# nanoporetech/medaka

Measured on NVIDIA H100. Metric: pileup positions/sec (consensus inference), higher is better.
Workload: dtype f32

## Files before the change

### medaka_b200/csrc/gru_wg.cu

```cuda
#include "common.cuh"
#include "ptx.cuh"
#include "rec_common.cuh"

namespace mdk {

constexpr int RW_THREADS = 256;
constexpr int RW_ABLK = (H / 8) * 64 * 16;
constexpr int RW_XBLK = 2 * 64 * 16;

template <int NT, bool FUSE_X, int OUT>
struct RwCfg {
    static constexpr int N = NT * RT_N;
    static constexpr bool HL = NT == 1;
    static constexpr int ROWS = HL ? 2 * N : N;
    static constexpr int PLANES = HL ? 1 : 2;
    static constexpr int KG = ROWS * 16 + 16;
    static constexpr int HPLANE = (H / 8) * KG;
    static constexpr int XPLANE = 2 * KG;
    static constexpr int HLO = HL ? N * 16 : HPLANE;
    static constexpr int XLO = HL ? N * 16 : XPLANE;
    static constexpr int RED = (RW_THREADS / 32) * NCLS * N;
    static constexpr int wlo_off = 0;
    static constexpr int wxlo_off = wlo_off + 6 * RW_ABLK;
    static constexpr int h_off = wxlo_off + (FUSE_X ? 6 * RW_XBLK : 0);
    static constexpr int x_off = h_off + 2 * PLANES * HPLANE;
    static constexpr int red_off = x_off + (FUSE_X ? 2 * PLANES * XPLANE : 0);
    static constexpr int total = red_off + (OUT == OUT_LOGITS ? 2 * RED * 4 : 0);
    static_assert(total <= 227 * 1024, "smem budget");
};

__device__ __forceinline__ uint32_t ld_u32(const __half *p) { return *reinterpret_cast<const uint32_t *>(p); }

template <int NT, bool FUSE_X, int OUT>
__global__ void __launch_bounds__(RW_THREADS, 1)
rec_tc_kernel(const float *__restrict__ gi, RecX xin, const __half *__restrict__ w_hh, const float *__restrict__ b_hn,
              void *__restrict__ h_out, int64_t B, int64_t T, const float *__restrict__ lin_w,
              float *__restrict__ plog) {
    using L = RwCfg<NT, FUSE_X, OUT>;
    constexpr int N = L::N, NA = N / 2;
    constexpr int NACC = L::ROWS / 2;
    constexpr int NX = FUSE_X ? NACC : NA;
    using MMA = Wgmma<N>;
    using MMA_H = Wgmma<L::ROWS>;
    constexpr bool LOGITS = OUT == OUT_LOGITS;
    extern __shared__ __align__(128) uint8_t smem[];
    const int tid = threadIdx.x, wg = tid >> 7, warp = (tid >> 5) & 3, lane = tid & 31;
    const int gq = lane >> 2, cq = lane & 3;
    const int dir = blockIdx.y;
    const int64_t ntiles = (B + RT_N - 1) / RT_N;
    const int64_t wtile0 = (int64_t)blockIdx.x * NT;
    const int j0 = wg * 64 + warp * 16 + gq;
    const uint32_t sbase = smem_u32(smem);

    for (int i = tid; i < (L::total - L::h_off) / 16; i += RW_THREADS)
        reinterpret_cast<int4 *>(smem + L::h_off)[i] = make_int4(0, 0, 0, 0);
    for (int i = tid; i < 3 * H * (H / 8); i += RW_THREADS) {
        const int kg = i & 15, r = (i >> 4) & (H - 1), gate = i >> 11;
        const uint4 v = *reinterpret_cast<const uint4 *>(w_hh + ((((size_t)dir * 2 + 1) * 3 + gate) * H + r) * H + kg * 8);
        *reinterpret_cast<uint4 *>(smem + L::wlo_off + (gate * 2 + (r >> 6)) * RW_ABLK + kg * 1024 + (r & 63) * 16) = v;
    }
    if (FUSE_X) {
        for (int i = tid; i < 3 * H * 2; i += RW_THREADS) {
            const int kg = i & 1, r = (i >> 1) & (H - 1), gate = i >> 8;
            const uint4 v = *reinterpret_cast<const uint4 *>(xin.w_x + ((((size_t)dir * 2 + 1) * 3 + gate) * H + r) * 16 + kg * 8);
            *reinterpret_cast<uint4 *>(smem + L::wxlo_off + (gate * 2 + (r >> 6)) * RW_XBLK + kg * 1024 + (r & 63) * 16) = v;
        }
    }
    float wlin[2][NCLS];
    if (LOGITS) {
#pragma unroll
        for (int hb = 0; hb < 2; ++hb)
#pragma unroll
            for (int c = 0; c < NCLS; ++c) wlin[hb][c] = lin_w[c * H2 + dir * H + j0 + 8 * hb];
    }
    uint32_t whi[3][H / 16][4];
#pragma unroll
    for (int gate = 0; gate < 3; ++gate)
#pragma unroll
        for (int ks = 0; ks < H / 16; ++ks) {
            const __half *w = w_hh + ((((size_t)dir * 2) * 3 + gate) * H + j0) * H + ks * 16 + 2 * cq;
            whi[gate][ks][0] = ld_u32(w);
            whi[gate][ks][1] = ld_u32(w + 8 * H);
            whi[gate][ks][2] = ld_u32(w + 8);
            whi[gate][ks][3] = ld_u32(w + 8 * H + 8);
        }
    uint32_t wxhi[3][4];
    float bx[3][2] = {};
    if (FUSE_X) {
#pragma unroll
        for (int gate = 0; gate < 3; ++gate) {
            const __half *w = xin.w_x + ((((size_t)dir * 2) * 3 + gate) * H + j0) * 16 + 2 * cq;
            wxhi[gate][0] = ld_u32(w);
            wxhi[gate][1] = ld_u32(w + 8 * 16);
            wxhi[gate][2] = ld_u32(w + 8);
            wxhi[gate][3] = ld_u32(w + 8 * 16 + 8);
            bx[gate][0] = xin.bias[dir * G3 + gate * H + j0];
            bx[gate][1] = xin.bias[dir * G3 + gate * H + j0 + 8];
        }
    }
    const float bhn[2] = {b_hn[dir * H + j0], b_hn[dir * H + j0 + 8]};

    float ar[NACC], az[NACC], an[NACC], axn[NX], hp[NA];
#pragma unroll
    for (int k = 0; k < NA; ++k) hp[k] = 0.f;
    auto load_pre = [&](int64_t t) {
#pragma unroll
        for (int i = 0; i < N / 8; ++i)
#pragma unroll
            for (int hb = 0; hb < 2; ++hb) {
                float2 v[3] = {make_float2(0.f, 0.f), make_float2(0.f, 0.f), make_float2(0.f, 0.f)};
                if (FUSE_X) {
#pragma unroll
                    for (int gate = 0; gate < 3; ++gate) v[gate] = make_float2(bx[gate][hb], bx[gate][hb]);
                } else if (wtile0 + (i >> 1) < ntiles) {
                    const float *p = gi + ((wtile0 + (i >> 1)) * T + t) * GI_TS_FLOATS +
                                     (((dir * 3) * 4 + 2 * (i & 1) + (cq >> 1)) * H + j0 + 8 * hb) * 4 + 2 * (cq & 1);
#pragma unroll
                    for (int gate = 0; gate < 3; ++gate) v[gate] = __ldcs(reinterpret_cast<const float2 *>(p + gate * 16 * H));
                }
                const int k = 4 * i + 2 * hb;
                ar[k] = v[0].x; ar[k + 1] = v[0].y;
                az[k] = v[1].x; az[k + 1] = v[1].y;
                axn[k] = v[2].x; axn[k + 1] = v[2].y;
                an[k] = bhn[hb]; an[k + 1] = bhn[hb];
            }
        if constexpr (L::HL) {
#pragma unroll
            for (int k = NA; k < NACC; ++k) {
                ar[k] = 0.f; az[k] = 0.f; an[k] = 0.f;
                if constexpr (FUSE_X) axn[k] = 0.f;
            }
        }
    };
    const int xF = FUSE_X ? xin.F : 1;
    const float *xsrc[NT];
    int xoff[NT];
    float xreg[NT];
#pragma unroll
    for (int m = 0; m < NT; ++m) {
        const int q = tid + RW_THREADS * m, xn = q / xF, xf = q - xn * xF;
        const bool own = FUSE_X && q < N * xF;
        xoff[m] = own ? (xf >> 3) * L::KG + xn * 16 + (xf & 7) * 2 : -1;
        xsrc[m] = (own && wtile0 * RT_N + xn < B) ? xin.feats + ((wtile0 * RT_N + xn) * T) * xF + xf : nullptr;
        xreg[m] = 0.f;
    }
    auto stage_x = [&](int buf, int m, float v) {
        __half hi, lo;
        split_f16(v, hi, lo);
        *reinterpret_cast<__half *>(smem + L::x_off + buf * L::PLANES * L::XPLANE + xoff[m]) = hi;
        *reinterpret_cast<__half *>(smem + L::x_off + buf * L::PLANES * L::XPLANE + L::XLO + xoff[m]) = lo;
    };
    const int64_t t_first = dir ? T - 1 : 0;
    if (FUSE_X) {
#pragma unroll
        for (int m = 0; m < NT; ++m) {
            if (xoff[m] < 0) continue;
            stage_x(0, m, xsrc[m] ? xsrc[m][t_first * xF] : 0.f);
            if (xsrc[m] && T > 1) xreg[m] = xsrc[m][(dir ? T - 2 : 1) * xF];
        }
    }
    load_pre(t_first);
    fence_proxy_async_smem();
    __syncthreads();

    constexpr int NW = N / 4;
    auto head_partials = [&](int rb) {
        float v[NW][NCLS];
#pragma unroll
        for (int wl = 0; wl < NW; ++wl) {
            const int k = 4 * (wl >> 1) + (wl & 1);
#pragma unroll
            for (int c = 0; c < NCLS; ++c) v[wl][c] = fmaf(wlin[1][c], hp[k + 2], wlin[0][c] * hp[k]);
        }
        int wbase = 0;
#pragma unroll
        for (int lvl = 0; lvl < 3; ++lvl) {
            const int mask = 16 >> lvl;
            const int half = (NW >> lvl) / 2;
            if (half > 0) {
                const bool up = lane & mask;
#pragma unroll
                for (int w = 0; w < NW / 2; ++w) {
                    if (w >= half) continue;
#pragma unroll
                    for (int c = 0; c < NCLS; ++c) {
                        const float send = up ? v[w][c] : v[w + half][c];
                        const float keep = up ? v[w + half][c] : v[w][c];
                        v[w][c] = keep + __shfl_xor_sync(0xffffffffu, send, mask);
                    }
                }
                if (up) wbase += half;
            } else {
#pragma unroll
                for (int c = 0; c < NCLS; ++c) v[0][c] += __shfl_xor_sync(0xffffffffu, v[0][c], mask);
            }
        }
        if (NW >= 8 || !(lane & 4)) {
            float *red = reinterpret_cast<float *>(smem + L::red_off) + rb * L::RED + (tid >> 5) * NCLS * N;
            const int n = 8 * (wbase >> 1) + 2 * cq + (wbase & 1);
#pragma unroll
            for (int c = 0; c < NCLS; ++c) red[c * N + n] = v[0][c];
        }
    };
    auto head_store = [&](int rb, int64_t t) {
        if (tid >= NCLS * N) return;
        const int c = tid / N, n = tid % N;
        const float *red = reinterpret_cast<const float *>(smem + L::red_off) + rb * L::RED + c * N + n;
        float s = red[0];
#pragma unroll
        for (int w = 1; w < RW_THREADS / 32; ++w) s += red[w * NCLS * N];
        const int64_t wt = wtile0 + n / RT_N;
        if (wt < ntiles) plog[((dir * ntiles + wt) * T + t) * PLOG_TS_FLOATS + c * RT_N + (n & 15)] = s;
    };

#pragma unroll 1
    for (int64_t step = 0; step < T; ++step) {
        const int64_t t = dir ? T - 1 - step : step;
        const int buf = (int)(step & 1);
        const uint32_t hb_addr = sbase + L::h_off + buf * L::PLANES * L::HPLANE;
        wg_fence();
        if constexpr (L::HL) {
#pragma unroll
            for (int ks = 0; ks < H / 16; ++ks) {
                const uint64_t bh = make_smem_desc(hb_addr + ks * 2 * L::KG, L::KG, 128);
#pragma unroll
                for (int gate = 0; gate < 3; ++gate) MMA_H::rs(gate == 0 ? ar : (gate == 1 ? az : an), whi[gate][ks], bh, 1u);
#pragma unroll
                for (int gate = 0; gate < 3; ++gate)
                    MMA::ss(gate == 0 ? ar : (gate == 1 ? az : an),
                            make_smem_desc(sbase + L::wlo_off + (gate * 2 + wg) * RW_ABLK + ks * 2 * 1024, 1024, 128), bh, 1u);
            }
        } else {
#pragma unroll
            for (int gate = 0; gate < 3; ++gate) {
                float(&acc)[NACC] = gate == 0 ? ar : (gate == 1 ? az : an);
#pragma unroll
                for (int ks = 0; ks < H / 16; ++ks) {
                    const uint64_t bh = make_smem_desc(hb_addr + ks * 2 * L::KG, L::KG, 128);
                    MMA::rs(acc, whi[gate][ks], bh, 1u);
                    MMA::rs(acc, whi[gate][ks], make_smem_desc(hb_addr + L::HPLANE + ks * 2 * L::KG, L::KG, 128), 1u);
                    MMA::ss(acc, make_smem_desc(sbase + L::wlo_off + (gate * 2 + wg) * RW_ABLK + ks * 2 * 1024, 1024, 128), bh, 1u);
                }
            }
        }
        if constexpr (FUSE_X) {
            const uint32_t xa = sbase + L::x_off + buf * L::PLANES * L::XPLANE;
            const uint64_t bh = make_smem_desc(xa, L::KG, 128);
            if constexpr (L::HL) {
#pragma unroll
                for (int gate = 0; gate < 3; ++gate) MMA_H::rs(gate == 0 ? ar : (gate == 1 ? az : axn), wxhi[gate], bh, 1u);
#pragma unroll
                for (int gate = 0; gate < 3; ++gate)
                    MMA::ss(gate == 0 ? ar : (gate == 1 ? az : axn),
                            make_smem_desc(sbase + L::wxlo_off + (gate * 2 + wg) * RW_XBLK, 1024, 128), bh, 1u);
            } else {
                const uint64_t bl = make_smem_desc(xa + L::XPLANE, L::KG, 128);
#pragma unroll
                for (int gate = 0; gate < 3; ++gate) {
                    float(&acc)[NACC] = gate == 0 ? ar : (gate == 1 ? az : axn);
                    MMA::rs(acc, wxhi[gate], bh, 1u);
                    MMA::rs(acc, wxhi[gate], bl, 1u);
                    MMA::ss(acc, make_smem_desc(sbase + L::wxlo_off + (gate * 2 + wg) * RW_XBLK, 1024, 128), bh, 1u);
                }
            }
        }
        wg_commit();
        if (!FUSE_X && tid == 0 && step + GI_PREFETCH_STEPS < T) {
            const int64_t tp = dir ? t - GI_PREFETCH_STEPS : t + GI_PREFETCH_STEPS;
#pragma unroll
            for (int m = 0; m < NT; ++m) {
                if (wtile0 + m >= ntiles) break;
                const float *blk = gi + ((wtile0 + m) * T + tp) * GI_TS_FLOATS + (int64_t)dir * (GI_TS_FLOATS / 2);
#pragma unroll
                for (int i = 0; i < 12; ++i) bulk_prefetch_l2(blk + i * 512, 2048);
            }
        }
        if (LOGITS && step > 0) {
            if (step > 1) head_store((int)((step - 1) & 1), dir ? t + 2 : t - 2);
            head_partials((int)(step & 1));
        }
        wg_wait_all();
        wg_hold(ar); wg_hold(az); wg_hold(an); wg_hold(axn);

        uint8_t *hw = smem + L::h_off + (buf ^ 1) * L::PLANES * L::HPLANE;
#pragma unroll
        for (int k = 0; k < NA; ++k) {
            float pr = ar[k], pz = az[k], pn = an[k], px = axn[k], r, z;
            if constexpr (L::HL) {
                pr += ar[k + NA]; pz += az[k + NA]; pn += an[k + NA];
                if constexpr (FUSE_X) px += axn[k + NA];
                const float a = 1.f + ex2_approx(fminf(pr, EXP_CLAMP)), b = 1.f + ex2_approx(fminf(pz, EXP_CLAMP));
                const float q = rcp_approx(a * b);
                r = b * q;
                z = a * q;
            } else {
                r = rcp_approx(1.f + ex2_approx(fminf(pr, EXP_CLAMP)));
                z = rcp_approx(1.f + ex2_approx(fminf(pz, EXP_CLAMP)));
            }
            const float en = ex2_approx(fminf(fmaf(r, pn, px), EXP_CLAMP));
            const float n = (en - 1.f) * rcp_approx(en + 1.f);
            hp[k] = fmaf(z, hp[k] - n, n);
            const int j = j0 + 8 * ((k >> 1) & 1), col = 8 * (k >> 2) + 2 * cq + (k & 1);
            __half hi, lo;
            split_f16(hp[k], hi, lo);
            *reinterpret_cast<__half *>(hw + (j >> 3) * L::KG + col * 16 + (j & 7) * 2) = hi;
            *reinterpret_cast<__half *>(hw + L::HLO + (j >> 3) * L::KG + col * 16 + (j & 7) * 2) = lo;
        }
        if (FUSE_X && step + 1 < T) {
#pragma unroll
            for (int m = 0; m < NT; ++m) {
                if (xoff[m] < 0) continue;
                stage_x(buf ^ 1, m, xreg[m]);
                if (xsrc[m] && step + 2 < T) xreg[m] = xsrc[m][(dir ? t - 2 : t + 2) * xF];
            }
        }
        if (!LOGITS) {
#pragma unroll
            for (int k = 0; k < NA; ++k) {
                const int i = k >> 2, n = 8 * i + 2 * cq + (k & 1);
                const int64_t wt = wtile0 + (i >> 1);
                if (wt >= ntiles) continue;
                const int64_t orow = (wt * T + t) * RT_N + (n & 15);
                const int kcol = dir * H + j0 + 8 * ((k >> 1) & 1);
                if (OUT == OUT_TILES) {
                    __half hi, lo;
                    split_f16(hp[k], hi, lo);
                    __half *o = reinterpret_cast<__half *>(reinterpret_cast<uint8_t *>(h_out) + (orow >> 7) * (int64_t)XT_TILE_BYTES +
                                                           (kcol >> 3) * (XT_ROWS * 16) + (orow & (XT_ROWS - 1)) * 16) + (kcol & 7);
                    o[0] = hi;
                    o[XT_PLANE_BYTES / 2] = lo;
                } else {
                    reinterpret_cast<float *>(h_out)[orow * H2 + kcol] = hp[k];
                }
            }
        }
        if (step + 1 < T) load_pre(dir ? t - 1 : t + 1);
        fence_proxy_async_smem();
        __syncthreads();
    }
    if (LOGITS) {
        if (T > 1) head_store((int)((T - 1) & 1), dir ? 1 : T - 2);
        head_partials((int)(T & 1));
        __syncthreads();
        head_store((int)(T & 1), dir ? 0 : T - 1);
    }
}

template <int NT, bool FX, int OUT>
static cudaError_t launch_rec(const float *gi, const RecX &xin, const __half *w_hh_tm, const float *b_hn, void *out,
                              const float *lin_w, int64_t B, int64_t T, cudaStream_t s) {
    auto kern = rec_tc_kernel<NT, FX, OUT>;
    constexpr int smem_bytes = RwCfg<NT, FX, OUT>::total;
    cudaError_t e = cudaFuncSetAttribute(kern, cudaFuncAttributeMaxDynamicSharedMemorySize, smem_bytes);
    if (e != cudaSuccess) return e;
    const int64_t tiles = (B + RT_N - 1) / RT_N;
    dim3 grid((unsigned)((tiles + NT - 1) / NT), NDIR);
    constexpr bool LOGITS = OUT == OUT_LOGITS;
    kern<<<grid, RW_THREADS, smem_bytes, s>>>(gi, xin, w_hh_tm, b_hn, LOGITS ? nullptr : out, B, T, lin_w,
                                              LOGITS ? static_cast<float *>(out) : nullptr);
    return cudaGetLastError();
}

template <int NT>
static cudaError_t launch_rec_nt(const float *gi, const RecX *xin, const __half *w_hh_tm, const float *b_hn, int out_kind,
                                 void *out, const float *lin_w, int64_t B, int64_t T, cudaStream_t s) {
    if (xin)
        return out_kind == OUT_TILES ? launch_rec<NT, true, OUT_TILES>(gi, *xin, w_hh_tm, b_hn, out, nullptr, B, T, s)
                                     : cudaErrorInvalidValue;
    const RecX none{nullptr, nullptr, nullptr, 0};
    switch (out_kind) {
    case OUT_TILES: return launch_rec<NT, false, OUT_TILES>(gi, none, w_hh_tm, b_hn, out, nullptr, B, T, s);
    case OUT_ROWS: return launch_rec<NT, false, OUT_ROWS>(gi, none, w_hh_tm, b_hn, out, nullptr, B, T, s);
    case OUT_LOGITS:
        return lin_w ? launch_rec<NT, false, OUT_LOGITS>(gi, none, w_hh_tm, b_hn, out, lin_w, B, T, s) : cudaErrorInvalidValue;
    }
    return cudaErrorInvalidValue;
}

cudaError_t launch_rec_tc(const float *gi, const RecX *xin, const __half *w_hh_tm, const float *b_hn, int tiles_per_cta,
                          int out_kind, void *out, const float *lin_w, int64_t B, int64_t T, cudaStream_t s) {
    if (B == 0 || T == 0) return cudaSuccess;
    switch (tiles_per_cta) {
    case 1: return launch_rec_nt<1>(gi, xin, w_hh_tm, b_hn, out_kind, out, lin_w, B, T, s);
    case 2: return launch_rec_nt<2>(gi, xin, w_hh_tm, b_hn, out_kind, out, lin_w, B, T, s);
    }
    return cudaErrorInvalidValue;
}

constexpr int GW_THREADS = 256;
constexpr int GW_QK = 8;
constexpr int GW_STAGE_PLANE = GW_QK * XT_ROWS * 16;
constexpr int GW_STAGE = 2 * GW_STAGE_PLANE;
constexpr int GW_NQ = XT_K / 8 / GW_QK;
constexpr int GW_X_OFF = XT_TILE_BYTES;
constexpr int GW_BAR_OFF = GW_X_OFF + 2 * GW_STAGE;
constexpr int GW_SMEM = GW_BAR_OFF + 16;

__global__ void __launch_bounds__(GW_THREADS, 1)
gemm_tc_kernel(const uint8_t *__restrict__ x_tiles, const __half *__restrict__ w_in_tm, const float *__restrict__ bias,
               float *__restrict__ gi, int64_t P, int64_t ntiles) {
    extern __shared__ __align__(128) uint8_t smem[];
    uint64_t *full = reinterpret_cast<uint64_t *>(smem + GW_BAR_OFF);
    const int tid = threadIdx.x, wg = tid >> 7, warp = (tid >> 5) & 3, lane = tid & 31;
    const int gq = lane >> 2, cq = lane & 3;
    const int blk = blockIdx.x;
    const uint32_t sbase = smem_u32(smem);
    for (int i = tid; i < 2 * H * (H2 / 8); i += GW_THREADS) {
        const int kg = i & 31, r = (i >> 5) & (H - 1), p = i >> 12;
        const uint4 v = reinterpret_cast<const uint4 *>(w_in_tm + (((size_t)blk * 2 + p) * H + r) * H2)[kg];
        *reinterpret_cast<uint4 *>(smem + p * XT_PLANE_BYTES + kg * (XT_ROWS * 16) + r * 16) = v;
    }
    if (tid == 0) {
        mbar_init(&full[0], 1);
        mbar_init(&full[1], 1);
        fence_mbar_init();
    }
    fence_proxy_async_smem();
    __syncthreads();
    const int64_t my_tiles = blockIdx.y < ntiles ? (ntiles - 1 - blockIdx.y) / gridDim.y + 1 : 0;
    const int64_t nst = my_tiles * GW_NQ;
    auto issue = [&](int64_t it) {
        const int64_t tile = blockIdx.y + (it / GW_NQ) * gridDim.y;
        const int q = (int)(it % GW_NQ), s = (int)(it & 1);
        const uint8_t *src = x_tiles + tile * (int64_t)XT_TILE_BYTES + q * GW_STAGE_PLANE;
        mbar_arrive_expect_tx(&full[s], GW_STAGE);
        bulk_g2s(smem + GW_X_OFF + s * GW_STAGE, src, GW_STAGE_PLANE, &full[s]);
        bulk_g2s(smem + GW_X_OFF + s * GW_STAGE + GW_STAGE_PLANE, src + XT_PLANE_BYTES, GW_STAGE_PLANE, &full[s]);
    };
    if (tid == 0) {
        if (nst > 0) issue(0);
        if (nst > 1) issue(1);
    }
    const float bj[2] = {bias[blk * H + wg * 64 + warp * 16 + gq], bias[blk * H + wg * 64 + warp * 16 + gq + 8]};
    float acc[64];
#pragma unroll 1
    for (int64_t it = 0; it < nst; ++it) {
        const int q = (int)(it % GW_NQ), s = (int)(it & 1);
        mbar_wait(&full[s], (uint32_t)((it >> 1) & 1));
        wg_fence();
#pragma unroll
        for (int prod = 0; prod < 3; ++prod) {
            const int pa = prod == 2, pb = prod == 1;
#pragma unroll
            for (int kk = 0; kk < GW_QK / 2; ++kk) {
                const uint64_t a = make_smem_desc(sbase + pa * XT_PLANE_BYTES + (q * GW_QK + 2 * kk) * (XT_ROWS * 16) + wg * 64 * 16,
                                                  XT_ROWS * 16, 128);
                const uint64_t b = make_smem_desc(sbase + GW_X_OFF + s * GW_STAGE + pb * GW_STAGE_PLANE + 2 * kk * (XT_ROWS * 16),
                                                  XT_ROWS * 16, 128);
                Wgmma<128>::ss(acc, a, b, (q | prod | kk) ? 1u : 0u);
            }
        }
        wg_commit();
        wg_wait_all();
        wg_hold(acc);
        __syncthreads();
        if (tid == 0 && it + 2 < nst) issue(it + 2);
        if (q == GW_NQ - 1) {
            const int64_t tile = blockIdx.y + (it / GW_NQ) * gridDim.y;
            const int64_t prem = P - tile * XT_ROWS;
#pragma unroll
            for (int k = 0; k < 64; k += 2) {
                const int c = 8 * (k >> 2) + 2 * cq, hb = (k >> 1) & 1;
                if (c >= prem) continue;
                const int j = wg * 64 + warp * 16 + gq + 8 * hb;
                float *o = gi + ((((tile * (XT_ROWS / WT) + (c >> 4)) * 6 + blk) * 4 + ((c & 15) >> 2)) * H + j) * 4 + (c & 3);
                __stcs(reinterpret_cast<float2 *>(o), make_float2(acc[k] + bj[hb], acc[k + 1] + bj[hb]));
            }
        }
    }
}

cudaError_t launch_gemm_tc(const void *x_tiles, const __half *w_in_tm, const float *bias, float *gi, int64_t P,
                           int sm_count, cudaStream_t s) {
    if (P == 0) return cudaSuccess;
    const int64_t ntiles = (P + XT_ROWS - 1) / XT_ROWS;
    cudaError_t ea = cudaFuncSetAttribute(gemm_tc_kernel, cudaFuncAttributeMaxDynamicSharedMemorySize, GW_SMEM);
    if (ea != cudaSuccess) return ea;
    int64_t ct = sm_count / 6;
    if (ct < 1) ct = 1;
    if (ct > ntiles) ct = ntiles;
    dim3 grid(6, (unsigned)ct);
    gemm_tc_kernel<<<grid, GW_THREADS, GW_SMEM, s>>>(reinterpret_cast<const uint8_t *>(x_tiles), w_in_tm, bias, gi, P, ntiles);
    return cudaGetLastError();
}

__global__ void __launch_bounds__(256, 1)
selftest_kernel(const float *__restrict__ A, const float *__restrict__ Bm, float *__restrict__ D, int N, int K) {
    extern __shared__ __align__(128) uint8_t smem[];
    const int a_plane = 128 * K * 2, b_plane = N * K * 2;
    uint8_t *sa = smem, *sb = smem + 2 * a_plane;
    const int tid = threadIdx.x, wg = tid >> 7, warp = (tid >> 5) & 3, lane = tid & 31;
    for (int i = tid; i < 128 * K; i += 256) {
        const int r = i / K, k = i % K;
        __half hi, lo;
        split_f16(A[i], hi, lo);
        const int off = (k / 8) * (128 * 16) + r * 16 + (k % 8) * 2;
        *reinterpret_cast<__half *>(sa + off) = hi;
        *reinterpret_cast<__half *>(sa + a_plane + off) = lo;
    }
    for (int i = tid; i < N * K; i += 256) {
        const int r = i / K, k = i % K;
        __half hi, lo;
        split_f16(Bm[i], hi, lo);
        const int off = (k / 8) * (N * 16) + r * 16 + (k % 8) * 2;
        *reinterpret_cast<__half *>(sb + off) = hi;
        *reinterpret_cast<__half *>(sb + b_plane + off) = lo;
    }
    fence_proxy_async_smem();
    __syncthreads();
    for (int n0 = 0; n0 < N; n0 += 16) {
        float d[8];
        wg_fence();
        uint32_t acc = 0;
        for (int prod = 0; prod < 3; ++prod) {
            const int pa = (prod == 2), pb = (prod == 1);
            for (int ks = 0; ks < K / 16; ++ks) {
                const uint64_t ad = make_smem_desc(smem_u32(sa + pa * a_plane) + ks * 2 * 128 * 16 + wg * 64 * 16, 128 * 16, 128);
                const uint64_t bd = make_smem_desc(smem_u32(sb + pb * b_plane) + ks * 2 * N * 16 + n0 * 16, N * 16, 128);
                Wgmma<16>::ss(d, ad, bd, acc);
                acc = 1;
            }
        }
        wg_commit();
        wg_wait_all();
        wg_hold(d);
        const int row = wg * 64 + warp * 16 + (lane >> 2);
        for (int k = 0; k < 8; ++k)
            D[(row + 8 * ((k >> 1) & 1)) * N + n0 + 8 * (k >> 2) + 2 * (lane & 3) + (k & 1)] = d[k];
    }
}

int selftest_umma(int device, const float *A, const float *B, float *D, int N, int K, int variant) {
    MDK_REQUIRE(N >= 16 && N <= 128 && N % 16 == 0, MDK_ERR_ARG, "selftest_umma: N must be a multiple of 16 in [16,128]");
    MDK_REQUIRE(K >= 16 && K <= 256 && K % 16 == 0, MDK_ERR_ARG, "selftest_umma: K must be a multiple of 16 in [16,256]");
    MDK_REQUIRE(variant == 0, MDK_ERR_ARG, "selftest_umma: variant must be 0");
    MDK_CUDA(cudaSetDevice(device));
    float *dA = nullptr, *dB = nullptr, *dD = nullptr;
    MDK_CUDA(cudaMalloc(&dA, sizeof(float) * 128 * K));
    MDK_CUDA(cudaMalloc(&dB, sizeof(float) * N * K));
    MDK_CUDA(cudaMalloc(&dD, sizeof(float) * 128 * N));
    MDK_CUDA(cudaMemcpy(dA, A, sizeof(float) * 128 * K, cudaMemcpyHostToDevice));
    MDK_CUDA(cudaMemcpy(dB, B, sizeof(float) * N * K, cudaMemcpyHostToDevice));
    const int smem = 2 * 128 * K * 2 + 2 * N * K * 2;
    MDK_REQUIRE(smem <= 227 * 1024, MDK_ERR_ARG, "selftest_umma: N*K too large for shared memory");
    MDK_CUDA(cudaFuncSetAttribute(selftest_kernel, cudaFuncAttributeMaxDynamicSharedMemorySize, smem));
    selftest_kernel<<<1, 256, smem>>>(dA, dB, dD, N, K);
    MDK_CUDA(cudaGetLastError());
    MDK_CUDA(cudaDeviceSynchronize());
    MDK_CUDA(cudaMemcpy(D, dD, sizeof(float) * 128 * N, cudaMemcpyDeviceToHost));
    cudaFree(dA); cudaFree(dB); cudaFree(dD);
    return MDK_OK;
}

}
```

### medaka_b200/csrc/ptx.cuh

```cuda
#pragma once
#include <cstdint>
#include <cuda_fp16.h>

namespace mdk {

__device__ __forceinline__ uint32_t smem_u32(const void *p) {
    return static_cast<uint32_t>(__cvta_generic_to_shared(p));
}

__device__ __forceinline__ void mbar_init(uint64_t *bar, uint32_t count) {
    asm volatile("mbarrier.init.shared::cta.b64 [%0], %1;" ::"r"(smem_u32(bar)), "r"(count) : "memory");
}
__device__ __forceinline__ void fence_mbar_init() {
    asm volatile("fence.mbarrier_init.release.cluster;" ::: "memory");
}
__device__ __forceinline__ void mbar_arrive_expect_tx(uint64_t *bar, uint32_t bytes) {
    asm volatile("mbarrier.arrive.expect_tx.shared::cta.b64 _, [%0], %1;" ::"r"(smem_u32(bar)), "r"(bytes)
                 : "memory");
}
__device__ __forceinline__ bool mbar_try_wait(uint64_t *bar, uint32_t parity) {
    uint32_t ok;
    asm volatile(
        "{\n\t.reg .pred p;\n\t"
        "mbarrier.try_wait.parity.shared::cta.b64 p, [%1], %2;\n\t"
        "selp.u32 %0, 1, 0, p;\n\t}"
        : "=r"(ok)
        : "r"(smem_u32(bar)), "r"(parity)
        : "memory");
    return ok != 0;
}
__device__ __forceinline__ void mbar_wait(uint64_t *bar, uint32_t parity) {
    if (mbar_try_wait(bar, parity)) return;
    const long long t0 = clock64();
    while (!mbar_try_wait(bar, parity)) {
        if (clock64() - t0 > 4000000000LL) __trap();
    }
}

__device__ __forceinline__ void fence_proxy_async_smem() {
    asm volatile("fence.proxy.async.shared::cta;" ::: "memory");
}

__device__ __forceinline__ uint32_t cluster_ctarank() {
    uint32_t r;
    asm volatile("mov.u32 %0, %%cluster_ctarank;" : "=r"(r));
    return r;
}
__device__ __forceinline__ uint32_t mapa_shared(uint32_t smem_addr, uint32_t rank) {
    uint32_t r;
    asm volatile("mapa.shared::cluster.u32 %0, %1, %2;" : "=r"(r) : "r"(smem_addr), "r"(rank));
    return r;
}
__device__ __forceinline__ void st_cluster_u32(uint32_t cluster_addr, uint32_t v) {
    asm volatile("st.shared::cluster.u32 [%0], %1;" ::"r"(cluster_addr), "r"(v) : "memory");
}
__device__ __forceinline__ void fence_proxy_async_cluster() {
    asm volatile("fence.proxy.async.shared::cluster;" ::: "memory");
}
__device__ __forceinline__ void mbar_arrive_cluster(uint32_t cluster_addr) {
    asm volatile("mbarrier.arrive.release.cluster.shared::cluster.b64 _, [%0];" ::"r"(cluster_addr) : "memory");
}
__device__ __forceinline__ bool mbar_try_wait_cluster(uint64_t *bar, uint32_t parity) {
    uint32_t ok;
    asm volatile(
        "{\n\t.reg .pred p;\n\t"
        "mbarrier.try_wait.parity.acquire.cluster.shared::cta.b64 p, [%1], %2;\n\t"
        "selp.u32 %0, 1, 0, p;\n\t}"
        : "=r"(ok)
        : "r"(smem_u32(bar)), "r"(parity)
        : "memory");
    return ok != 0;
}
__device__ __forceinline__ void mbar_wait_cluster(uint64_t *bar, uint32_t parity) {
    if (mbar_try_wait_cluster(bar, parity)) return;
    const long long t0 = clock64();
    while (!mbar_try_wait_cluster(bar, parity)) {
        if (clock64() - t0 > 4000000000LL) __trap();
    }
}
__device__ __forceinline__ void cluster_sync_all() {
    asm volatile("barrier.cluster.arrive.release.aligned;\n\tbarrier.cluster.wait.acquire.aligned;" ::: "memory");
}
__device__ __forceinline__ void named_bar_sync(uint32_t id, uint32_t count) {
    asm volatile("bar.sync %0, %1;" ::"r"(id), "r"(count) : "memory");
}

__device__ __forceinline__ void bulk_prefetch_l2(const void *gmem_src, uint32_t bytes) {
    asm volatile("cp.async.bulk.prefetch.L2.global [%0], %1;" ::"l"(gmem_src), "r"(bytes) : "memory");
}

__device__ __forceinline__ void bulk_g2s(void *smem_dst, const void *gmem_src, uint32_t bytes, uint64_t *bar) {
    asm volatile(
        "cp.async.bulk.shared::cluster.global.mbarrier::complete_tx::bytes [%0], [%1], %2, [%3];" ::"r"(
            smem_u32(smem_dst)),
        "l"(gmem_src), "r"(bytes), "r"(smem_u32(bar))
        : "memory");
}

__device__ __forceinline__ uint64_t make_smem_desc(uint32_t smem_addr, uint32_t lbo_bytes, uint32_t sbo_bytes) {
    uint64_t d = 0;
    d |= static_cast<uint64_t>((smem_addr & 0x3FFFF) >> 4);
    d |= static_cast<uint64_t>((lbo_bytes >> 4) & 0x3FFF) << 16;
    d |= static_cast<uint64_t>((sbo_bytes >> 4) & 0x3FFF) << 32;
    return d;
}
__device__ __forceinline__ void wg_fence() { asm volatile("wgmma.fence.sync.aligned;" ::: "memory"); }
__device__ __forceinline__ void wg_commit() { asm volatile("wgmma.commit_group.sync.aligned;" ::: "memory"); }
__device__ __forceinline__ void wg_wait_all() { asm volatile("wgmma.wait_group.sync.aligned 0;" ::: "memory"); }
template <int R>
__device__ __forceinline__ void wg_hold(float (&d)[R]) {
#pragma unroll
    for (int i = 0; i < R; ++i) asm volatile("" : "+f"(d[i])::"memory");
}

template <int N> struct Wgmma;
template <> struct Wgmma<16> {
    __device__ __forceinline__ static void ss(float (&d)[8], uint64_t a, uint64_t b, uint32_t accumulate) {
        asm volatile(
            "{\n\t.reg .pred p;\n\tsetp.ne.b32 p, %10, 0;\n\t"
            "wgmma.mma_async.sync.aligned.m64n16k16.f32.f16.f16 {%0,%1,%2,%3,%4,%5,%6,%7}, %8, %9, p, 1, 1, 0, 0;\n\t}"
            : "+f"(d[0]), "+f"(d[1]), "+f"(d[2]), "+f"(d[3]), "+f"(d[4]), "+f"(d[5]), "+f"(d[6]), "+f"(d[7])
            : "l"(a), "l"(b), "r"(accumulate));
    }
    __device__ __forceinline__ static void rs(float (&d)[8], const uint32_t (&a)[4], uint64_t b, uint32_t accumulate) {
        asm volatile(
            "{\n\t.reg .pred p;\n\tsetp.ne.b32 p, %13, 0;\n\t"
            "wgmma.mma_async.sync.aligned.m64n16k16.f32.f16.f16 {%0,%1,%2,%3,%4,%5,%6,%7}, {%8,%9,%10,%11}, %12, p, 1, 1, 0;\n\t}"
            : "+f"(d[0]), "+f"(d[1]), "+f"(d[2]), "+f"(d[3]), "+f"(d[4]), "+f"(d[5]), "+f"(d[6]), "+f"(d[7])
            : "r"(a[0]), "r"(a[1]), "r"(a[2]), "r"(a[3]), "l"(b), "r"(accumulate));
    }
    __device__ __forceinline__ static void ss(float (&d)[16], uint64_t a, uint64_t b, uint32_t accumulate) {
        asm volatile(
            "{\n\t.reg .pred p;\n\tsetp.ne.b32 p, %10, 0;\n\t"
            "wgmma.mma_async.sync.aligned.m64n16k16.f32.f16.f16 {%0,%1,%2,%3,%4,%5,%6,%7}, %8, %9, p, 1, 1, 0, 0;\n\t}"
            : "+f"(d[0]), "+f"(d[1]), "+f"(d[2]), "+f"(d[3]), "+f"(d[4]), "+f"(d[5]), "+f"(d[6]), "+f"(d[7])
            : "l"(a), "l"(b), "r"(accumulate));
    }
};
template <> struct Wgmma<32> {
    __device__ __forceinline__ static void ss(float (&d)[16], uint64_t a, uint64_t b, uint32_t accumulate) {
        asm volatile(
            "{\n\t.reg .pred p;\n\tsetp.ne.b32 p, %18, 0;\n\t"
            "wgmma.mma_async.sync.aligned.m64n32k16.f32.f16.f16 {%0,%1,%2,%3,%4,%5,%6,%7,%8,%9,%10,%11,%12,%13,%14,%15}, %16, %17, p, 1, 1, 0, 0;\n\t}"
            : "+f"(d[0]), "+f"(d[1]), "+f"(d[2]), "+f"(d[3]), "+f"(d[4]), "+f"(d[5]), "+f"(d[6]), "+f"(d[7]),
              "+f"(d[8]), "+f"(d[9]), "+f"(d[10]), "+f"(d[11]), "+f"(d[12]), "+f"(d[13]), "+f"(d[14]), "+f"(d[15])
            : "l"(a), "l"(b), "r"(accumulate));
    }
    __device__ __forceinline__ static void rs(float (&d)[16], const uint32_t (&a)[4], uint64_t b, uint32_t accumulate) {
        asm volatile(
            "{\n\t.reg .pred p;\n\tsetp.ne.b32 p, %21, 0;\n\t"
            "wgmma.mma_async.sync.aligned.m64n32k16.f32.f16.f16 {%0,%1,%2,%3,%4,%5,%6,%7,%8,%9,%10,%11,%12,%13,%14,%15}, {%16,%17,%18,%19}, %20, p, 1, 1, 0;\n\t}"
            : "+f"(d[0]), "+f"(d[1]), "+f"(d[2]), "+f"(d[3]), "+f"(d[4]), "+f"(d[5]), "+f"(d[6]), "+f"(d[7]),
              "+f"(d[8]), "+f"(d[9]), "+f"(d[10]), "+f"(d[11]), "+f"(d[12]), "+f"(d[13]), "+f"(d[14]), "+f"(d[15])
            : "r"(a[0]), "r"(a[1]), "r"(a[2]), "r"(a[3]), "l"(b), "r"(accumulate));
    }
};
template <> struct Wgmma<128> {
    __device__ __forceinline__ static void ss(float (&d)[64], uint64_t a, uint64_t b, uint32_t accumulate) {
        asm volatile(
            "{\n\t.reg .pred p;\n\tsetp.ne.b32 p, %66, 0;\n\t"
            "wgmma.mma_async.sync.aligned.m64n128k16.f32.f16.f16 {%0,%1,%2,%3,%4,%5,%6,%7,%8,%9,%10,%11,%12,%13,%14,%15,%16,%17,%18,%19,%20,%21,%22,%23,%24,%25,%26,%27,%28,%29,%30,%31,%32,%33,%34,%35,%36,%37,%38,%39,%40,%41,%42,%43,%44,%45,%46,%47,%48,%49,%50,%51,%52,%53,%54,%55,%56,%57,%58,%59,%60,%61,%62,%63}, %64, %65, p, 1, 1, 0, 0;\n\t}"
            : "+f"(d[0]), "+f"(d[1]), "+f"(d[2]), "+f"(d[3]), "+f"(d[4]), "+f"(d[5]), "+f"(d[6]), "+f"(d[7]),
              "+f"(d[8]), "+f"(d[9]), "+f"(d[10]), "+f"(d[11]), "+f"(d[12]), "+f"(d[13]), "+f"(d[14]), "+f"(d[15]),
              "+f"(d[16]), "+f"(d[17]), "+f"(d[18]), "+f"(d[19]), "+f"(d[20]), "+f"(d[21]), "+f"(d[22]), "+f"(d[23]),
              "+f"(d[24]), "+f"(d[25]), "+f"(d[26]), "+f"(d[27]), "+f"(d[28]), "+f"(d[29]), "+f"(d[30]), "+f"(d[31]),
              "+f"(d[32]), "+f"(d[33]), "+f"(d[34]), "+f"(d[35]), "+f"(d[36]), "+f"(d[37]), "+f"(d[38]), "+f"(d[39]),
              "+f"(d[40]), "+f"(d[41]), "+f"(d[42]), "+f"(d[43]), "+f"(d[44]), "+f"(d[45]), "+f"(d[46]), "+f"(d[47]),
              "+f"(d[48]), "+f"(d[49]), "+f"(d[50]), "+f"(d[51]), "+f"(d[52]), "+f"(d[53]), "+f"(d[54]), "+f"(d[55]),
              "+f"(d[56]), "+f"(d[57]), "+f"(d[58]), "+f"(d[59]), "+f"(d[60]), "+f"(d[61]), "+f"(d[62]), "+f"(d[63])
            : "l"(a), "l"(b), "r"(accumulate));
    }
};

__device__ __forceinline__ void split_f16(float v, __half &hi, __half &lo) {
    hi = __float2half_rn(v);
    lo = __float2half_rn(v - __half2float(hi));
}

__device__ __forceinline__ float ldg_stream(const float *p) {
    float v;
    asm volatile("ld.global.nc.L1::no_allocate.f32 %0, [%1];" : "=f"(v) : "l"(p));
    return v;
}

__device__ __forceinline__ float4 ld_stream4(const float *p) {
    float4 v;
    asm volatile("ld.global.nc.L1::no_allocate.v4.f32 {%0,%1,%2,%3}, [%4];"
                 : "=f"(v.x), "=f"(v.y), "=f"(v.z), "=f"(v.w)
                 : "l"(p));
    return v;
}

}
```

Baseline: 116.1 million.

## Deepen input-GEMM TMA pipeline to three stages and overlap wgmma groups

The input-projection GEMM kernel now uses three shared-memory stages for the bulk-copied x tiles instead of two, and it restructures the loop per tile over K chunks. wgmma groups are kept in flight with wait_group 1 rather than draining after every chunk, so a chunk's math overlaps the next chunk's issue, and a stage is refilled as soon as its group retires. This is meant to hide TMA latency and tensor-core drain bubbles in the input GEMM. It costs extra shared memory and more complex stage and parity bookkeeping, and there is some risk around the ordering of smem reuse.

```diff
diff --git a/medaka_b200/csrc/gru_wg.cu b/medaka_b200/csrc/gru_wg.cu
--- a/medaka_b200/csrc/gru_wg.cu
+++ b/medaka_b200/csrc/gru_wg.cu
@@ -392,9 +392,11 @@
 constexpr int GW_STAGE_PLANE = GW_QK * XT_ROWS * 16;
 constexpr int GW_STAGE = 2 * GW_STAGE_PLANE;
 constexpr int GW_NQ = XT_K / 8 / GW_QK;
+constexpr int GW_NS = 3;
 constexpr int GW_X_OFF = XT_TILE_BYTES;
-constexpr int GW_BAR_OFF = GW_X_OFF + 2 * GW_STAGE;
-constexpr int GW_SMEM = GW_BAR_OFF + 16;
+constexpr int GW_BAR_OFF = GW_X_OFF + GW_NS * GW_STAGE;
+constexpr int GW_SMEM = GW_BAR_OFF + GW_NS * 8;
+static_assert(GW_SMEM <= 227 * 1024, "smem budget");
 
 __global__ void __launch_bounds__(GW_THREADS, 1)
 gemm_tc_kernel(const uint8_t *__restrict__ x_tiles, const __half *__restrict__ w_in_tm, const float *__restrict__ bias,
@@ -411,8 +413,7 @@
         *reinterpret_cast<uint4 *>(smem + p * XT_PLANE_BYTES + kg * (XT_ROWS * 16) + r * 16) = v;
     }
     if (tid == 0) {
-        mbar_init(&full[0], 1);
-        mbar_init(&full[1], 1);
+        for (int i = 0; i < GW_NS; ++i) mbar_init(&full[i], 1);
         fence_mbar_init();
     }
     fence_proxy_async_smem();
@@ -421,51 +422,57 @@
     const int64_t nst = my_tiles * GW_NQ;
     auto issue = [&](int64_t it) {
         const int64_t tile = blockIdx.y + (it / GW_NQ) * gridDim.y;
-        const int q = (int)(it % GW_NQ), s = (int)(it & 1);
+        const int q = (int)(it % GW_NQ), s = (int)(it % GW_NS);
         const uint8_t *src = x_tiles + tile * (int64_t)XT_TILE_BYTES + q * GW_STAGE_PLANE;
         mbar_arrive_expect_tx(&full[s], GW_STAGE);
         bulk_g2s(smem + GW_X_OFF + s * GW_STAGE, src, GW_STAGE_PLANE, &full[s]);
         bulk_g2s(smem + GW_X_OFF + s * GW_STAGE + GW_STAGE_PLANE, src + XT_PLANE_BYTES, GW_STAGE_PLANE, &full[s]);
     };
-    if (tid == 0) {
-        if (nst > 0) issue(0);
-        if (nst > 1) issue(1);
-    }
+    if (tid == 0)
+        for (int i = 0; i < GW_NS && i < nst; ++i) issue(i);
     const float bj[2] = {bias[blk * H + wg * 64 + warp * 16 + gq], bias[blk * H + wg * 64 + warp * 16 + gq + 8]};
     float acc[64];
 #pragma unroll 1
-    for (int64_t it = 0; it < nst; ++it) {
-        const int q = (int)(it % GW_NQ), s = (int)(it & 1);
-        mbar_wait(&full[s], (uint32_t)((it >> 1) & 1));
-        wg_fence();
-#pragma unroll
-        for (int prod = 0; prod < 3; ++prod) {
-            const int pa = prod == 2, pb = prod == 1;
-#pragma unroll
-            for (int kk = 0; kk < GW_QK / 2; ++kk) {
-                const uint64_t a = make_smem_desc(sbase + pa * XT_PLANE_BYTES + (q * GW_QK + 2 * kk) * (XT_ROWS * 16) + wg * 64 * 16,
-                                                  XT_ROWS * 16, 128);
-                const uint64_t b = make_smem_desc(sbase + GW_X_OFF + s * GW_STAGE + pb * GW_STAGE_PLANE + 2 * kk * (XT_ROWS * 16),
-                                                  XT_ROWS * 16, 128);
-                Wgmma<128>::ss(acc, a, b, (q | prod | kk) ? 1u : 0u);
-            }
-        }
-        wg_commit();
-        wg_wait_all();
+    for (int64_t ti = 0; ti < my_tiles; ++ti) {
+#pragma unroll
+        for (int q = 0; q < GW_NQ; ++q) {
+            const int64_t it = ti * GW_NQ + q;
+            const int s = (int)(it % GW_NS);
+            mbar_wait(&full[s], (uint32_t)((it / GW_NS) & 1));
+            wg_fence();
+#pragma unroll
+            for (int prod = 0; prod < 3; ++prod) {
+                const int pa = prod == 2, pb = prod == 1;
+#pragma unroll
+                for (int kk = 0; kk < GW_QK / 2; ++kk) {
+                    const uint64_t a = make_smem_desc(sbase + pa * XT_PLANE_BYTES + (q * GW_QK + 2 * kk) * (XT_ROWS * 16) + wg * 64 * 16,
+                                                      XT_ROWS * 16, 128);
+                    const uint64_t b = make_smem_desc(sbase + GW_X_OFF + s * GW_STAGE + pb * GW_STAGE_PLANE + 2 * kk * (XT_ROWS * 16),
+                                                      XT_ROWS * 16, 128);
+                    Wgmma<128>::ss(acc, a, b, (q | prod | kk) ? 1u : 0u);
+                }
+            }
+            wg_commit();
+            if (q > 0) {
+                wg_wait<1>();
+                __syncthreads();
+                if (tid == 0 && it + GW_NS - 1 < nst) issue(it + GW_NS - 1);
+            }
+        }
+        wg_wait<0>();
         wg_hold(acc);
         __syncthreads();
-        if (tid == 0 && it + 2 < nst) issue(it + 2);
-        if (q == GW_NQ - 1) {
-            const int64_t tile = blockIdx.y + (it / GW_NQ) * gridDim.y;
-            const int64_t prem = P - tile * XT_ROWS;
-#pragma unroll
-            for (int k = 0; k < 64; k += 2) {
-                const int c = 8 * (k >> 2) + 2 * cq, hb = (k >> 1) & 1;
-                if (c >= prem) continue;
-                const int j = wg * 64 + warp * 16 + gq + 8 * hb;
-                float *o = gi + ((((tile * (XT_ROWS / WT) + (c >> 4)) * 6 + blk) * 4 + ((c & 15) >> 2)) * H + j) * 4 + (c & 3);
-                __stcs(reinterpret_cast<float2 *>(o), make_float2(acc[k] + bj[hb], acc[k + 1] + bj[hb]));
-            }
+        const int64_t it_last = ti * GW_NQ + GW_NQ - 1;
+        if (tid == 0 && it_last + GW_NS < nst) issue(it_last + GW_NS);
+        const int64_t tile = blockIdx.y + ti * gridDim.y;
+        const int64_t prem = P - tile * XT_ROWS;
+#pragma unroll
+        for (int k = 0; k < 64; k += 2) {
+            const int c = 8 * (k >> 2) + 2 * cq, hb = (k >> 1) & 1;
+            if (c >= prem) continue;
+            const int j = wg * 64 + warp * 16 + gq + 8 * hb;
+            float *o = gi + ((((tile * (XT_ROWS / WT) + (c >> 4)) * 6 + blk) * 4 + ((c & 15) >> 2)) * H + j) * 4 + (c & 3);
+            __stcs(reinterpret_cast<float2 *>(o), make_float2(acc[k] + bj[hb], acc[k + 1] + bj[hb]));
         }
     }
 }
diff --git a/medaka_b200/csrc/ptx.cuh b/medaka_b200/csrc/ptx.cuh
--- a/medaka_b200/csrc/ptx.cuh
+++ b/medaka_b200/csrc/ptx.cuh
@@ -107,6 +107,8 @@
 __device__ __forceinline__ void wg_fence() { asm volatile("wgmma.fence.sync.aligned;" ::: "memory"); }
 __device__ __forceinline__ void wg_commit() { asm volatile("wgmma.commit_group.sync.aligned;" ::: "memory"); }
 __device__ __forceinline__ void wg_wait_all() { asm volatile("wgmma.wait_group.sync.aligned 0;" ::: "memory"); }
+template <int N>
+__device__ __forceinline__ void wg_wait() { asm volatile("wgmma.wait_group.sync.aligned %0;" ::"n"(N) : "memory"); }
 template <int R>
 __device__ __forceinline__ void wg_hold(float (&d)[R]) {
 #pragma unroll
```

New measurement: 116.6 million, median of 6. No clear change (+0.4%).
